# RoyAPTX4869/RaLD

Hardware: AMD Instinct MI355X
Metric: denoising steps/sec (whole node) (higher is better)
Workload: dtype bf16

## Files before the change

### include/rald_hip.h

```cpp
#ifndef RALD_HIP_H
#define RALD_HIP_H
#include <stdint.h>
#ifdef __cplusplus
extern "C" {
#endif

const char* rald_last_error(void);
int rald_version(void);
int rald_build_flags(void);
int64_t rald_debug_f16_saturation_count(int32_t reset);
int rald_debug_poison_lds(void* stream);

typedef struct rald_dit rald_dit;

typedef struct rald_dit_config {
    int32_t n_latents;
    int32_t channels;
    int32_t depth;
    int32_t n_heads;
    int32_t d_head;
    int32_t t_channels;
    int32_t context_dim;
    int32_t n_cond_tokens;
    int32_t with_radar_enc;
// ... 158 lines not shown
int64_t rald_radar_points_workspace_bytes(const rald_radar_points_config* cfg, int32_t batch);
int rald_radar_points_run(const rald_radar_points* h, const float* cubes, int32_t batch, float* points, int32_t* counts, int32_t* peaks,
                          float* intensities, void* workspace, int64_t workspace_bytes, void* stream);

typedef struct rald_lidar_config {
    double pc_range[6];
    double voxel_size[3];
    int32_t max_points_per_voxel, max_voxels, num_point_features;
    int32_t view_cone_mode, norm_anisotropy, norm_isotropy;
    double extrinsic[16];
    double fov[6];
} rald_lidar_config;
typedef struct rald_lidar rald_lidar;
int rald_lidar_create(const rald_lidar_config* cfg, rald_lidar** out);
void rald_lidar_destroy(rald_lidar* h);
int64_t rald_lidar_workspace_bytes(const rald_lidar_config* cfg, int32_t batch, int64_t total_points);
int rald_lidar_crop(const rald_lidar* h, const float* points, int32_t in_stride, const int64_t* offsets, int32_t batch, float* out,
                    int32_t* counts, void* workspace, int64_t workspace_bytes, void* stream);
int rald_lidar_voxelize(const rald_lidar* h, const float* points, const int64_t* offsets, const int32_t* counts, int32_t batch,
                        int32_t to_polar, float* polar_out, float* voxels, int32_t* coords, int32_t* num_points, int32_t* kept_keys,
                        int32_t* voxel_counts, void* workspace, int64_t workspace_bytes, void* stream);
int rald_lidar_queries(const rald_lidar* h, const float* points, const int64_t* offsets, int32_t batch, int32_t num_samples,
                       int32_t in_num, const int64_t* sample_idx, const double* u_in, const int64_t* voxel_idx, const double* u_out,
                       const int64_t* empty_rank, const int32_t* coords, const int32_t* kept_keys, const int32_t* voxel_counts,
                       float* lidar_points, float* query_points, float* query_labels, void* workspace, int64_t workspace_bytes,
                       void* stream);

int rald_op_gemm_nt(const void* A, int64_t lda, int64_t strideA, const void* B, int64_t ldb, int64_t strideB,
                    void* C, int64_t ldc, int64_t strideC, const float* bias, int32_t M, int32_t N, int32_t K,
                    int32_t batch, float alpha, int32_t epilogue, void* stream);
int rald_op_gemm_nt2(const void* A, int64_t lda, int64_t strideA, int64_t strideA2, const void* B, int64_t ldb, int64_t strideB, int64_t strideB2,
                     void* C, int64_t ldc, int64_t strideC, int64_t strideC2, const float* bias, int32_t M, int32_t N, int32_t K, int32_t batch,
                     int32_t batch2, float alpha, int32_t epilogue, void* stream);
int rald_op_gemm_tn(const void* A_bf16, int64_t lda, const void* B_bf16, int64_t ldb, float* C, int64_t ldc, float* colsum, int32_t M, int32_t N1,
                    int32_t N2, void* workspace, int64_t workspace_bytes, void* stream);
int rald_op_conv3d_wgrad(const void* dy_bf16, const void* x_bf16, float* dW, float* dbias, int32_t B, int32_t ID, int32_t IH, int32_t IW, int32_t Cin,
                         int32_t Cout, int32_t stride, int32_t pad, void* workspace, int64_t workspace_bytes, void* stream);
int64_t rald_op_gemm_tn_workspace_bytes(int32_t M, int32_t N1, int32_t N2);
int64_t rald_op_conv3d_wgrad_workspace_bytes(int32_t B, int32_t ID, int32_t IH, int32_t IW, int32_t Cin, int32_t Cout, int32_t stride, int32_t pad);
int rald_op_patches27(const float* cube, int32_t cube_ch, void* out_bf16, int32_t B, int32_t D, int32_t H, int32_t W, void* stream);
int rald_op_transpose(const void* in, int32_t in_is_bf16, int64_t ld_in, int64_t stride_in, int64_t stride_in2, void* out_bf16, int64_t ld_out,
                      int64_t stride_out, int64_t stride_out2, int32_t rows, int32_t cols, int32_t batch, int32_t batch2, void* stream);
int rald_op_ln_mod_bwd(const float* x, const float* dh, const float* scale, int64_t gstride, int32_t rows_per_group, float add_one, float eps,
                       int64_t rows, int32_t D, float* dx_accum, void* dx_bf16_out, float* dscale_accum, float* dshift_accum, void* stream);
int rald_op_geglu_fwd(const void* u_bf16, void* hid_bf16, int64_t M, int32_t inner, void* stream);
int rald_op_geglu_bwd(const void* u_bf16, const void* dhid_bf16, void* du_bf16, int64_t M, int32_t inner, void* stream);
int rald_op_colsum(const void* X, int32_t is_bf16, int64_t ld, int64_t M, int32_t N, float* out_accum, void* stream);
int rald_op_row_lse(const float* S, int64_t rows, int32_t cols, float scale, float* lse, void* stream);
int rald_op_rowdot_heads(const void* dO_bf16, const void* O_bf16, int64_t M, int32_t heads, int32_t nq, float* delta, void* stream);
int rald_op_attn_bwd_elem(const float* S, const float* dP, const float* lse, const float* delta, int64_t batch, int32_t R, int32_t Ccols,
                          int64_t vbatch_stride, int32_t vstride, float scale, int32_t by_col, void* P_bf16, void* dS_bf16, void* stream);
int rald_op_sgemm_acc(const float* A, int64_t lda, int32_t trans_a, const float* B, int64_t ldb, int32_t trans_b, float* C, int64_t ldc, int32_t M,
                      int32_t N, int32_t K, float alpha, void* stream);
int rald_op_silu_fwd(const float* x, float* y, int64_t n, void* stream);
int rald_op_silu_bwd(const float* x_pre, const float* dy, float* dx, int64_t n, void* stream);
int rald_op_posemb(const float* t, float* out, int32_t n, int32_t channels, void* stream);
int rald_op_edm_loss_grad(const float* F, const float* x_noised, const float* y, const float* coef3, int64_t per_sample, int64_t total, float* dF,
                          float* D_out, double* loss, void* stream);
int rald_op_conv3d(const void* in_bf16, const void* w_packed_bf16, const float* bias, const float* resid, float* out, void* out_bf16, int32_t B,
                   int32_t ID, int32_t IH, int32_t IW, int32_t Cin, int32_t Cout, int32_t stride, int32_t pad, void* stream);
int rald_op_conv3d_route(int32_t B, int32_t ID, int32_t IH, int32_t IW, int32_t Cin, int32_t Cout, int32_t stride, int32_t pad, int32_t allow_split,
                         int32_t* splits_out);
int rald_op_conv3d_full(const void* in_bf16, const void* w_packed_bf16, const float* bias, const float* resid, float* out, void* out_bf16,
                        double* gn_part, void* split_workspace, int64_t split_workspace_bytes, int32_t allow_split, int32_t B, int32_t ID,
                        int32_t IH, int32_t IW, int32_t Cin, int32_t Cout, int32_t stride, int32_t pad, void* stream);
int rald_op_gn_finish(const double* part, double* stats, int32_t B, int32_t nblk, void* stream);
// ... 117 lines not shown
```

### rald_amd/_handles.py

```python
from __future__ import annotations

import ctypes as C
import os
from typing import Dict, Iterable, Optional, Sequence, Tuple

import torch

from . import _lib
from ._lib import DitConfig, check, lib


def _stream() -> int:
    return torch.cuda.current_stream().cuda_stream


def _opt(t: Optional[torch.Tensor]) -> Optional[int]:
    return t.data_ptr() if t is not None else None


def _need_cuda(t: torch.Tensor, what: str) -> None:
    if not t.is_cuda:
        raise RuntimeError(f"rald_amd: {what} must live on the GPU (cuda tensor); this package has no CPU path")


# ... 296 lines not shown
def op_philox_normal(seeds: torch.Tensor, n_per_sample: int, tag: int = 0, step: int = 0, out: Optional[torch.Tensor] = None) -> torch.Tensor:
    _need_cuda(seeds, "seeds")
    if seeds.dtype != torch.int64 or seeds.dim() != 1:
        raise ValueError("seeds must be an int64 [B] tensor")
    seeds = seeds.contiguous()
    B = seeds.shape[0]
    if out is None:
        out = torch.empty(B, int(n_per_sample), device=seeds.device, dtype=torch.float32)
    assert out.dtype == torch.float32 and out.is_cuda and out.is_contiguous() and out.numel() == B * int(n_per_sample)
    check(lib().rald_op_philox_normal(seeds.data_ptr(), B, int(n_per_sample), int(tag), int(step), out.data_ptr(), _stream()))
    return out


def op_gemm_nt(A: torch.Tensor, B: torch.Tensor, bias: Optional[torch.Tensor] = None, epilogue: int = 0,
               C_inout: Optional[torch.Tensor] = None, alpha: float = 1.0) -> torch.Tensor:
    batched = A.dim() == 3 or B.dim() == 3
    batch = (A.shape[0] if A.dim() == 3 else B.shape[0]) if batched else 1
    M, K = A.shape[-2], A.shape[-1]
    N = B.shape[-2]
    sA = A.stride(0) if A.dim() == 3 else 0
    sB = B.stride(0) if B.dim() == 3 else 0
    nc = N // 2 if epilogue == 3 else N
    if epilogue == 2:
        out = C_inout
    else:
        shape = (batch, M, nc) if batched else (M, nc)
        out = torch.empty(shape, device=A.device, dtype=torch.float16 if epilogue == 5 else (torch.bfloat16 if epilogue in (0, 3, 4) else torch.float32))
    sC = out.stride(0) if out.dim() == 3 else 0
    check(lib().rald_op_gemm_nt(A.data_ptr(), A.stride(-2), sA, B.data_ptr(), B.stride(-2), sB, out.data_ptr(), out.stride(-2), sC, _opt(bias), M, N,
                                K, batch, alpha, epilogue, _stream()))
    return out


def op_gemm_tn(A: torch.Tensor, B: torch.Tensor, C_inout: torch.Tensor, colsum: Optional[torch.Tensor] = None, atomics: bool = True) -> torch.Tensor:
    M, N1 = A.shape
    N2 = B.shape[1]
    assert A.dtype == torch.bfloat16 and B.dtype == torch.bfloat16 and C_inout.dtype == torch.float32 and B.shape[0] == M
    assert A.stride(1) == 1 and B.stride(1) == 1 and C_inout.stride(1) == 1 and C_inout.shape == (N1, N2)
    ws, nbytes = None, 0
    if not atomics:
        nbytes = lib().rald_op_gemm_tn_workspace_bytes(M, N1, N2)
        ws = _scratch(nbytes, A.device)
    check(lib().rald_op_gemm_tn(A.data_ptr(), A.stride(0), B.data_ptr(), B.stride(0), C_inout.data_ptr(), C_inout.stride(0),
                                _opt(colsum), M, N1, N2, _opt(ws), nbytes, _stream()))
    return C_inout


def op_gemm_resid_ln(A: torch.Tensor, W: torch.Tensor, bias: torch.Tensor, x: torch.Tensor, g: torch.Tensor, b: torch.Tensor,
                     gstride: int = 0, rows_per_group: int = 1 << 30, add_one: float = 0.0, eps: float = 1e-5) -> torch.Tensor:
    M, K = A.shape
    h = torch.empty(M, 512, device=A.device, dtype=torch.bfloat16)
    check(lib().rald_op_gemm_resid_ln(A.data_ptr(), A.stride(0), W.data_ptr(), W.stride(0), bias.data_ptr(),
                                      x.data_ptr(), h.data_ptr(), g.data_ptr(), b.data_ptr(), gstride,
                                      rows_per_group, add_one, eps, M, K, _stream()))
    return h


def op_resid_gemm_ln(x: torch.Tensor, bias: torch.Tensor, M: int, K: int, A: Optional[torch.Tensor] = None, W: Optional[torch.Tensor] = None,
                     A8: Optional[torch.Tensor] = None, SA: Optional[torch.Tensor] = None, W8: Optional[torch.Tensor] = None,
                     SW: Optional[torch.Tensor] = None, h: Optional[torch.Tensor] = None, h8: Optional[torch.Tensor] = None,
                     hs: Optional[torch.Tensor] = None, g: Optional[torch.Tensor] = None, b: Optional[torch.Tensor] = None, gstride: int = 0,
                     rows_per_group: int = 1 << 30, add_one: float = 0.0, eps: float = 1e-5, strideW: int = 0, w_rows: int = 0, nt_io: int = 1,
                     route: int = 0, scratch: Optional[torch.Tensor] = None, lda: Optional[int] = None, ldw: Optional[int] = None) -> None:
    a, w = (A, W) if A is not None else (A8, W8)
    lda = a.stride(-2) if lda is None else lda
    ldw = w.stride(-2) if ldw is None else ldw
# ... 343 lines not shown
```

### rald_amd/csrc/api.hip

```cpp
#include <cstdlib>
#include <cstring>

#include "ae.h"
#include "dit.h"
#include "lidar.h"
#include "radar_dsp.h"
#include "radar_points.h"

using namespace rald;

struct rald_dit { Dit impl; };
struct rald_ae { Ae impl; };

extern "C" {

const char* rald_last_error(void) { return rald::last_error(); }
int rald_version(void) { return 3; }
int rald_build_flags(void) { return 0; }

int64_t rald_debug_f16_saturation_count(int32_t reset) {
    unsigned a = 0, b = 0;
    if (hipDeviceSynchronize() != hipSuccess) return -1;
    if (f16_saturation_gemm(&a, reset != 0) || f16_saturation_attn(&b, reset != 0)) return -1;
    return (int64_t)a + (int64_t)b;
// ... 465 lines not shown
int rald_optim_clip_coef(const double* sumsq, float pre_scale, float max_norm, float* out_norm_coef, void* stream) {
    RALD_CHECK(sumsq && out_norm_coef, "rald_optim_clip_coef: null argument");
    return optim_clip_coef(sumsq, pre_scale, max_norm, out_norm_coef, (hipStream_t)stream);
}
int rald_optim_adamw_ema(float* params, const float* grads, float* exp_avg, float* exp_avg_sq, float* ema_params, int64_t n,
                         const float* grad_scale, double lr, double beta1, double beta2, double eps, double weight_decay, int64_t step,
                         double ema_rate, int32_t write_back_grads, void* stream) {
    RALD_CHECK(n == 0 || (params && grads && exp_avg && exp_avg_sq), "rald_optim_adamw_ema: null argument");
    return optim_adamw_ema(params, grads, exp_avg, exp_avg_sq, ema_params, n, grad_scale, lr, beta1, beta2, eps, weight_decay, step, ema_rate,
                           write_back_grads, (hipStream_t)stream);
}
int rald_optim_ema(float* ema_params, const float* params, int64_t n, double rate, void* stream) {
    RALD_CHECK(n == 0 || (ema_params && params), "rald_optim_ema: null argument");
    return optim_ema(ema_params, params, n, rate, (hipStream_t)stream);
}

int rald_op_gemm_nt(const void* A, int64_t lda, int64_t strideA, const void* B, int64_t ldb, int64_t strideB,
                    void* C, int64_t ldc, int64_t strideC, const float* bias, int32_t M, int32_t N, int32_t K,
                    int32_t batch, float alpha, int32_t epilogue, void* stream) {
    RALD_CHECK(A && B && C, "rald_op_gemm_nt: null pointer");
    GemmArgs g;
    g.A = (const bf16*)A; g.lda = lda; g.strideA = strideA; g.B = (const bf16*)B; g.ldb = ldb; g.strideB = strideB;
    g.C = C; g.ldc = ldc; g.strideC = strideC; g.bias = bias; g.M = M; g.N = N; g.K = K; g.batch = batch; g.alpha = alpha; g.alpha_ncols = 1 << 30; g.flags = 0;
    return gemm_nt(g, epilogue, (hipStream_t)stream);
}
int rald_op_gemm_nt2(const void* A, int64_t lda, int64_t strideA, int64_t strideA2, const void* B, int64_t ldb, int64_t strideB, int64_t strideB2,
                     void* C, int64_t ldc, int64_t strideC, int64_t strideC2, const float* bias, int32_t M, int32_t N, int32_t K, int32_t batch,
                     int32_t batch2, float alpha, int32_t epilogue, void* stream) {
    RALD_CHECK(A && B && C, "rald_op_gemm_nt2: null pointer");
    GemmArgs g = gemm_args((const bf16*)A, lda, (const bf16*)B, ldb, C, ldc, bias, M, N, K);
    g.strideA = strideA; g.strideB = strideB; g.strideC = strideC; g.batch = batch; g.alpha = alpha;
    g.batch2 = batch2; g.strideA2 = strideA2; g.strideB2 = strideB2; g.strideC2 = strideC2;
    return gemm_nt(g, epilogue, (hipStream_t)stream);
}
int rald_op_gemm_tn(const void* A_bf16, int64_t lda, const void* B_bf16, int64_t ldb, float* C, int64_t ldc, float* colsum, int32_t M, int32_t N1,
                    int32_t N2, void* workspace, int64_t workspace_bytes, void* stream) {
    return gemm_tn((const bf16*)A_bf16, lda, (const bf16*)B_bf16, ldb, C, ldc, colsum, M, N1, N2, (hipStream_t)stream, (float*)workspace, workspace_bytes / 4);
}
int rald_op_conv3d_wgrad(const void* dy_bf16, const void* x_bf16, float* dW, float* dbias, int32_t B, int32_t ID, int32_t IH, int32_t IW, int32_t Cin,
                         int32_t Cout, int32_t stride, int32_t pad, void* workspace, int64_t workspace_bytes, void* stream) {
    return conv3d_wgrad_tn((const bf16*)dy_bf16, (const bf16*)x_bf16, dW, dbias, B, ID, IH, IW, Cin, Cout, stride, pad, (hipStream_t)stream, (float*)workspace,
                           workspace_bytes / 4);
}
int64_t rald_op_gemm_tn_workspace_bytes(int32_t M, int32_t N1, int32_t N2) { return 4 * gemm_tn_workspace_floats(M, N1, N2); }
int64_t rald_op_conv3d_wgrad_workspace_bytes(int32_t B, int32_t ID, int32_t IH, int32_t IW, int32_t Cin, int32_t Cout, int32_t stride, int32_t pad) {
    return 4 * conv3d_wgrad_workspace_floats(B, ID, IH, IW, Cin, Cout, stride, pad);
}
int rald_op_patches27(const float* cube, int32_t cube_ch, void* out_bf16, int32_t B, int32_t D, int32_t H, int32_t W, void* stream) {
    return patches27(cube, cube_ch, (bf16*)out_bf16, B, D, H, W, (hipStream_t)stream);
}
int rald_op_transpose(const void* in, int32_t in_is_bf16, int64_t ld_in, int64_t stride_in, int64_t stride_in2, void* out_bf16, int64_t ld_out,
                      int64_t stride_out, int64_t stride_out2, int32_t rows, int32_t cols, int32_t batch, int32_t batch2, void* stream) {
    TransposeArgs a;
    a.in = in; a.ld_in = ld_in; a.stride_in = stride_in; a.stride_in2 = stride_in2; a.out = (bf16*)out_bf16; a.ld_out = ld_out;
    a.stride_out = stride_out; a.stride_out2 = stride_out2; a.rows = rows; a.cols = cols; a.batch = batch; a.batch2 = batch2;
    return transpose_rows(a, in_is_bf16, (hipStream_t)stream);
}
int rald_op_ln_mod_bwd(const float* x, const float* dh, const float* scale, int64_t gstride, int32_t rows_per_group, float add_one, float eps,
                       int64_t rows, int32_t D, float* dx_accum, void* dx_bf16_out, float* dscale_accum, float* dshift_accum, void* stream) {
    RALD_CHECK(x && dh && scale && dx_accum && dscale_accum && dshift_accum, "rald_op_ln_mod_bwd: null pointer");
    return ln_mod_bwd(x, dh, scale, gstride, rows_per_group, add_one, eps, rows, D, dx_accum, dscale_accum, dshift_accum, (hipStream_t)stream, (bf16*)dx_bf16_out);
}
int rald_op_geglu_fwd(const void* u_bf16, void* hid_bf16, int64_t M, int32_t inner, void* stream) {
    RALD_CHECK(u_bf16 && hid_bf16, "rald_op_geglu_fwd: null pointer");
    return geglu_fwd((const bf16*)u_bf16, (bf16*)hid_bf16, M, inner, (hipStream_t)stream);
}
// ... 377 lines not shown
```

### rald_amd/csrc/gemm.hip

```cpp
#include <cstdlib>
#include <type_traits>

#include "common.h"
#include "kernels.h"
#include "gemm_epilogue.h"
#include "gemm_tile.h"

namespace rald {

template <int MT, int NT, int EPI>
__device__ __forceinline__ void gemm_epilogue(f32x4 (&acc)[MT][NT], const GemmArgs& a, int mb, int nb, int64_t coff, int fr, int fq) {
    if constexpr (EPI == EPI_GEGLU) {
        bf16* C = reinterpret_cast<bf16*>(a.C) + coff;
#pragma unroll
        for (int i = 0; i < MT; ++i) {
            const int m = mb + i * 16 + fr;
            if (m >= a.M) continue;
#pragma unroll
            for (int p = 0; p < NT / 2; ++p) {
                const int nx = nb + 32 * p + 4 * fq;
                const int ng = nx + 16;
                float4 bx = *reinterpret_cast<const float4*>(a.bias + nx);
                float4 bg = *reinterpret_cast<const float4*>(a.bias + ng);
                f32x4 x = acc[i][2 * p], g = acc[i][2 * p + 1];
                bf16x4 o = pack4((x[0] + bx.x) * gelu_erf(g[0] + bg.x), (x[1] + bx.y) * gelu_erf(g[1] + bg.y),
                                 (x[2] + bx.z) * gelu_erf(g[2] + bg.z), (x[3] + bx.w) * gelu_erf(g[3] + bg.w));
                const int c = nb / 2 + 16 * p + 4 * fq;
                *reinterpret_cast<bf16x4*>(C + (int64_t)m * a.ldc + c) = o;
            }
        }
    } else {
#pragma unroll
// ... 248 lines not shown
            __builtin_amdgcn_s_barrier();
        };
        for (int kt = 1; kt + 1 < nk; ++kt) body(kt, std::true_type{});
        if (nk > 1) body(nk - 1, std::false_type{});
        mfma_all(fa1, fb1);
    } else {
#pragma unroll
        for (int s = 0; s < NSTAGE - 1; ++s)
            if (s < nk) stage(s, s);
        for (int kt = 0; kt < nk; ++kt) {
            if (kt + NSTAGE - 2 < nk) asm volatile("s_waitcnt vmcnt(%0)" ::"n"((NSTAGE - 2) * (CA + CB)) : "memory");
            else asm volatile("s_waitcnt vmcnt(0)" ::: "memory");
            asm volatile("" ::: "memory");
            __builtin_amdgcn_s_barrier();
            asm volatile("" ::: "memory");
            if (kt + NSTAGE - 1 < nk) stage(kt + NSTAGE - 1, (kt + NSTAGE - 1) % NSTAGE);
#pragma unroll
            for (int kk = 0; kk < 2; ++kk) {
                bf16x8 fa[MT], fb[NT];
                read_frags(kt % NSTAGE, kk, fa, fb);
                mfma_all(fa, fb);
            }
        }
    }
    if constexpr (NSTAGE != 2) {
        asm volatile("" ::: "memory");
        __builtin_amdgcn_s_barrier();
        asm volatile("" ::: "memory");
    }
    gemm_epilogue_lds<MT, NT, EPI>(acc, a, m0 + wm * (BM / WM), n0 + wn * (BN / WN), coff, lane, smem + wave * EPI_PATCH_BYTES,
                                   reinterpret_cast<float*>(smem + WAVES * EPI_PATCH_BYTES) + wave * NT * 16);
}

template <int BM, int BN>
static int launch_tile(const GemmArgs& a, int epi, hipStream_t st) {
    dim3 grid(cdiv(a.N, BN), cdiv(a.M, BM), a.batch * a.batch2);
    switch (epi) {
        case EPI_BF16:  hipLaunchKernelGGL((gemm_nt_kernel<BM, BN, EPI_BF16>), grid, dim3(256), 0, st, a); break;
        case EPI_F32:   hipLaunchKernelGGL((gemm_nt_kernel<BM, BN, EPI_F32>), grid, dim3(256), 0, st, a); break;
        case EPI_RESID: hipLaunchKernelGGL((gemm_nt_kernel<BM, BN, EPI_RESID>), grid, dim3(256), 0, st, a); break;
        case EPI_GEGLU: hipLaunchKernelGGL((gemm_nt_kernel<BM, BN, EPI_GEGLU>), grid, dim3(256), 0, st, a); break;
        default: set_error("gemm: bad epilogue"); return 1;
    }
    RALD_HIP(hipGetLastError());
    return 0;
}

template <int BM, int BN, int WM, int WN, int NSTAGE, int EPI>
static int launch_glds_epi(const GemmArgs& a, hipStream_t st) {
    constexpr int WAVES = WM * WN;
    constexpr int smem = NSTAGE * (BM + BN) * 64 * 2;
    static_assert(smem >= epi_lds_bytes<BN / (16 * WN)>(WAVES), "epilogue patches and bias slots must fit in the staging buffers");
    static bool raised = false;
    return launch_dyn_lds(gemm_nt_glds_kernel<BM, BN, WM, WN, NSTAGE, EPI>, raised, dim3(cdiv(a.N, BN), cdiv(a.M, BM), a.batch * a.batch2), WAVES * 64, smem, st, a);
}
template <int BM, int BN, int WM, int WN, int NSTAGE>
static int launch_glds(const GemmArgs& a, int epi, hipStream_t st) {
    switch (epi) {
        case EPI_BF16:  return launch_glds_epi<BM, BN, WM, WN, NSTAGE, EPI_BF16>(a, st);
        case EPI_F32:   return launch_glds_epi<BM, BN, WM, WN, NSTAGE, EPI_F32>(a, st);
        case EPI_RESID: return launch_glds_epi<BM, BN, WM, WN, NSTAGE, EPI_RESID>(a, st);
        case EPI_GEGLU: return launch_glds_epi<BM, BN, WM, WN, NSTAGE, EPI_GEGLU>(a, st);
        case EPI_F16S:
            if constexpr ((BM == 64 && BN == 64) || (BM == 128 && BN == 128 && NSTAGE == 2)) return launch_glds_epi<BM, BN, WM, WN, NSTAGE, EPI_F16S>(a, st);
            else { set_error("gemm: the fp16-slab epilogue is built for the 64x64 ring and the 128x128 LDS-DMA engines"); return 1; }
        case EPI_SOFTMAX64:
            if constexpr ((BN / WN) % 64 == 0 && BM >= 128) return launch_glds_epi<BM, BN, WM, WN, NSTAGE, EPI_SOFTMAX64>(a, st);
            else { set_error("gemm: the softmax epilogue needs waves of 64-column groups"); return 1; }
        default: set_error("gemm: bad epilogue"); return 1;
    }
}

int f16_saturation_gemm(unsigned* count, bool reset) {
    RALD_HIP(hipMemcpyFromSymbol(count, HIP_SYMBOL(g_f16_sat_gemm), sizeof(unsigned)));
    if (reset) { const unsigned z = 0; RALD_HIP(hipMemcpyToSymbol(HIP_SYMBOL(g_f16_sat_gemm), &z, sizeof(unsigned))); }
    return 0;
}

int gemm_nt(const GemmArgs& a0, int epi, hipStream_t st) {
    GemmArgs a = a0;
    a.flags |= GEMM_NT_STORE;
    RALD_CHECK(a.M > 0 && a.N > 0 && a.K > 0 && a.batch > 0 && a.batch2 > 0, "gemm: empty problem");
    const int64_t nbatch = (int64_t)a.batch * a.batch2;
    RALD_CHECK(nbatch <= 65535, "gemm: batch * batch2 exceeds the grid z limit");
    RALD_CHECK(a.K % 64 == 0, "gemm: K must be a multiple of 64 (pad with zeros)");
    RALD_CHECK(a.N % 4 == 0, "gemm: N must be a multiple of 4");
    RALD_CHECK(a.lda % 8 == 0 && a.ldb % 8 == 0, "gemm: lda/ldb must be multiples of 8 elements (16-byte rows)");
    RALD_CHECK(a.lda >= a.K && a.ldb >= a.K, "gemm: leading dimension smaller than K");
    RALD_CHECK(((uintptr_t)a.A % 16 == 0) && ((uintptr_t)a.B % 16 == 0) && ((uintptr_t)a.C % 16 == 0), "gemm: pointers must be 16-byte aligned");
    RALD_CHECK(a.ldc % 4 == 0, "gemm: ldc must be a multiple of 4");
    if (epi == EPI_GEGLU) {
        RALD_CHECK(a.N % 128 == 0 && a.bias != nullptr, "gemm: GEGLU needs N % 128 == 0 and a packed bias");
        RALD_CHECK(a.ldc >= a.N / 2, "gemm: GEGLU ldc < N/2");
    } else {
        RALD_CHECK(a.ldc >= a.N, "gemm: ldc < N");
    }
    if (epi == EPI_F16S) {
        RALD_CHECK(!a.out8 && a.N % 8 == 0, "gemm: the fp16-slab epilogue needs N % 8 == 0");
        const int64_t w128 = (int64_t)cdiv(a.M, 128) * cdiv(a.N, 128) * nbatch, w64 = (int64_t)cdiv(a.M, 64) * cdiv(a.N, 64) * nbatch;
        RALD_CHECK(w128 >= 192 || w64 <= 256, "gemm: fp16 slabs are not built for the register-staged engine (ask gemm_f16s_ok first)");
        if (w128 >= 192) return launch_glds<128, 128, 2, 2, 2>(a, epi, st);
        return launch_glds<64, 64, 2, 2, 8>(a, epi, st);
    }
    if (epi == EPI_SOFTMAX64) {
        RALD_CHECK(a.M % 128 == 0 && a.N % 128 == 0 && !a.bias && !a.out8 && a.alpha_ncols >= a.N, "gemm: the softmax epilogue needs M, N % 128 == 0 and no bias");
        if (a.M % 256 == 0 && a.N % 256 == 0 && (int64_t)(a.M / 256) * (a.N / 256) * nbatch >= 256) return launch_glds<256, 256, 4, 2, 2>(a, epi, st);
        return launch_glds<128, 128, 2, 2, 2>(a, epi, st);
    }
    if (a.out8) {
        RALD_CHECK(epi == EPI_GEGLU && a.outs && a.batch * a.batch2 == 1 && a.M % 256 == 0 && a.N % 256 == 0 && (a.N / 2) % 32 == 0 &&
                   (int64_t)(a.M / 256) * (a.N / 256) >= 256, "gemm: the MXFP8 output form needs the GEGLU epilogue on full 256x256 tiles");
        return launch_glds<256, 256, 4, 2, 2>(a, epi, st);
    }
    const int64_t wg128 = (int64_t)cdiv(a.M, 128) * cdiv(a.N, 128) * nbatch;
    if (wg128 < 192) {
        const int64_t wg64 = (int64_t)cdiv(a.M, 64) * cdiv(a.N, 64) * nbatch;
        if (wg64 > 256) return launch_tile<64, 64>(a, epi, st);
        return launch_glds<64, 64, 2, 2, 8>(a, epi, st);
    }
    const int64_t wg256 = (int64_t)(a.M / 256) * (a.N / 256) * nbatch;
    if (a.M % 256 == 0 && a.N % 256 == 0 && wg256 >= 256) return launch_glds<256, 256, 4, 2, 2>(a, epi, st);
    if (epi != EPI_GEGLU && wg128 <= 320 && a.M % 64 == 0) return launch_glds<64, 128, 2, 2, 3>(a, epi, st);
    return launch_glds<128, 128, 2, 2, 2>(a, epi, st);
}

}
```

### rald_amd/csrc/gemm_tile.h

```cpp
#pragma once
#include "common.h"

namespace rald {

typedef int i32x8 __attribute__((ext_vector_type(8)));
typedef int i32x4 __attribute__((ext_vector_type(4)));

#define RALD_SWZ(row, chunk) ((chunk) ^ ((row) & 7))

__device__ __forceinline__ void xcd_strip_tile(int& tm, int& tn) {
    const int ntn = gridDim.x, ntm = gridDim.y, nt = ntn * ntm;
    const int lin = blockIdx.y * gridDim.x + blockIdx.x;
    const int xcd = lin & 7, q = nt >> 3, rr = nt & 7;
    const int tile = (xcd < rr ? xcd * (q + 1) : rr * (q + 1) + (xcd - rr) * q) + (lin >> 3);
    constexpr int GN = 8;
    if (ntn % GN == 0) {
        const int strip = tile / (ntm * GN), within = tile % (ntm * GN);
        tm = within / GN;
        tn = strip * GN + within % GN;
    } else {
        tm = tile / ntn;
        tn = tile % ntn;
    }
}

template <int WAVES, typename T, int C>
__device__ __forceinline__ void dma_sources(const T* (&g)[C], const T* base, int64_t ld, int row0, int rows, int wave, int lane) {
    const int lr = lane >> 3;
    const int lc = RALD_SWZ(lr, lane & 7);
#pragma unroll
    for (int p = 0; p < C; ++p) {
        int r = row0 + 8 * (wave + WAVES * p) + lr;
        r = r < rows ? r : rows - 1;
        g[p] = base + (int64_t)r * ld + lc * (16 / (int)sizeof(T));
    }
}
template <int BM, int WAVES, typename T, int CA, int CB>
__device__ __forceinline__ void dma_stage(const T* const (&gA)[CA], const T* const (&gB)[CB], int kt, int nk, unsigned char* stage, int wave) {
    constexpr int BK = 128 / (int)sizeof(T);
    const int koff = 0;
    int ks = kt + koff;
    ks = ks >= nk ? ks - nk : ks;
#pragma unroll
    for (int p = 0; p < CA; ++p)
        __builtin_amdgcn_global_load_lds((glb_void*)(gA[p] + ks * BK), (lds_void*)(stage + (wave + WAVES * p) * 1024), 16, 0, 0);
#pragma unroll
    for (int p = 0; p < CB; ++p)
        __builtin_amdgcn_global_load_lds((glb_void*)(gB[p] + ks * BK), (lds_void*)(stage + BM * 128 + (wave + WAVES * p) * 1024), 16, 0, 0);
}

__device__ __forceinline__ i32x8 frag_mx8(const unsigned char* tile, int row, int fq) {
    const i32x4* s = reinterpret_cast<const i32x4*>(tile) + row * 8;
    const i32x4 lo = s[RALD_SWZ(row, fq)], hi = s[RALD_SWZ(row, fq + 4)];
    return i32x8{lo[0], lo[1], lo[2], lo[3], hi[0], hi[1], hi[2], hi[3]};
}

// ... 84 lines not shown
```

### rald_amd/csrc/kernels.h

```cpp
#pragma once
#include <cstdlib>
#include <vector>

#include "common.h"

namespace rald {

enum { GEMM_NT_STORE = 64 };
enum { EPI_BF16 = 0, EPI_F32 = 1, EPI_RESID = 2, EPI_GEGLU = 3,
       EPI_SOFTMAX64 = 4,
       EPI_F16S = 5 };
struct GemmArgs {
    const bf16* A; int64_t lda; int64_t strideA;
    const bf16* B; int64_t ldb; int64_t strideB;
    void* C;       int64_t ldc; int64_t strideC;
    const float* bias;
    int M, N, K, batch;
    float alpha;
    int alpha_ncols;
    int flags;
    int batch2 = 1;
    int64_t strideA2 = 0, strideB2 = 0, strideC2 = 0;
    unsigned char *out8 = nullptr, *outs = nullptr;
};
#ifdef __HIPCC__
__device__ __forceinline__ void gemm_batch_offsets(const GemmArgs& a, int bz, int64_t& oa, int64_t& ob, int64_t& oc) {
    const int b1 = bz / a.batch2, b2 = bz - b1 * a.batch2;
    oa = (int64_t)b1 * a.strideA + (int64_t)b2 * a.strideA2;
    ob = (int64_t)b1 * a.strideB + (int64_t)b2 * a.strideB2;
    oc = (int64_t)b1 * a.strideC + (int64_t)b2 * a.strideC2;
}
#endif
int gemm_nt(const GemmArgs& a, int epi, hipStream_t st);
int f16_saturation_gemm(unsigned* count, bool reset);
int f16_saturation_attn(unsigned* count, bool reset);
inline bool gemm_f16s_ok(int M, int N, int batch) {
    const int64_t w128 = (int64_t)((M + 127) / 128) * ((N + 127) / 128) * batch, w64 = (int64_t)((M + 63) / 64) * ((N + 63) / 64) * batch;
    return w128 >= 192 || w64 <= 256;
}
inline GemmArgs gemm_args(const bf16* A, int64_t lda, const bf16* B, int64_t ldb, void* C, int64_t ldc,
                          const float* bias, int M, int N, int K) {
    GemmArgs g;
    g.A = A; g.lda = lda; g.strideA = 0; g.B = B; g.ldb = ldb; g.strideB = 0;
    g.C = C; g.ldc = ldc; g.strideC = 0; g.bias = bias; g.M = M; g.N = N; g.K = K; g.batch = 1; g.alpha = 1.f; g.alpha_ncols = 1 << 30; g.flags = 0;
    return g;
}

struct GemmLnArgs {
    const bf16* A; int64_t lda;
    const bf16* W; int64_t ldw;
    const float* bias;
    float* x;
    bf16* h;
    unsigned char* h8 = nullptr;
    unsigned char* hs = nullptr;
    int nt_io = 1;
    const unsigned char *A8 = nullptr, *SA = nullptr, *W8 = nullptr, *SW = nullptr;
    const float* g; const float* b; int64_t gstride; int rows_per_group; float add_one, eps;
    int M, K;
    int64_t strideW = 0; int w_rows = 1 << 30;
};
int gemm_resid_ln(const GemmLnArgs& a, hipStream_t st);
inline bool gemm_resid_ln_pays(int M, int K = 512) { (void)K; return M >= 16384; }
inline GemmLnArgs gemm_ln_args(const bf16* A, int64_t lda, const bf16* W, int64_t ldw, const float* bias, float* x, bf16* h,
                               const float* g, const float* b, int64_t gstride, int rows_per_group, float add_one, int M, int K) {
    GemmLnArgs a;
// ... 270 lines not shown
```

Baseline: 5659.

## Add persistent 256x256 GEMM kernel that prefetches the next tile during the epilogue

Adds a persistent bf16 GEMM kernel (256x256 tiles, 8 waves, half of them issuing direct-to-LDS loads) that loops over output tiles. It starts loading the next tile's first K stages before running the current tile's epilogue, which stages output through LDS. gemm_nt routes single-batch BF16/GEGLU problems with at least two tiles per CU to this kernel instead of the non-persistent 256x256 path. This aims to remove per-tile launch and prologue cost and to hide epilogue stores behind the next tile's loads. In exchange it adds hand-scheduled code that needs a large LDS allocation, plus a test entry point.

```diff
diff --git a/include/rald_hip.h b/include/rald_hip.h
--- a/include/rald_hip.h
+++ b/include/rald_hip.h
@@ -214,6 +214,8 @@
 int rald_op_gemm_nt2(const void* A, int64_t lda, int64_t strideA, int64_t strideA2, const void* B, int64_t ldb, int64_t strideB, int64_t strideB2,
                      void* C, int64_t ldc, int64_t strideC, int64_t strideC2, const float* bias, int32_t M, int32_t N, int32_t K, int32_t batch,
                      int32_t batch2, float alpha, int32_t epilogue, void* stream);
+int rald_op_gemm_nt_256(const void* A, int64_t lda, const void* B, int64_t ldb, void* C, int64_t ldc, const float* bias, int32_t M, int32_t N,
+                        int32_t K, float alpha, int32_t alpha_ncols, int32_t epilogue, int32_t persistent, int32_t max_workgroups, void* stream);
 int rald_op_gemm_tn(const void* A_bf16, int64_t lda, const void* B_bf16, int64_t ldb, float* C, int64_t ldc, float* colsum, int32_t M, int32_t N1,
                     int32_t N2, void* workspace, int64_t workspace_bytes, void* stream);
 int rald_op_conv3d_wgrad(const void* dy_bf16, const void* x_bf16, float* dW, float* dbias, int32_t B, int32_t ID, int32_t IH, int32_t IW, int32_t Cin,
diff --git a/rald_amd/_handles.py b/rald_amd/_handles.py
--- a/rald_amd/_handles.py
+++ b/rald_amd/_handles.py
@@ -352,6 +352,16 @@
     return out
 
 
+def op_gemm_nt_256(A: torch.Tensor, B: torch.Tensor, out: torch.Tensor, bias: Optional[torch.Tensor] = None, epilogue: int = 0, alpha: float = 1.0,
+                   alpha_ncols: int = 1 << 30, persistent: int = 1, max_workgroups: int = 1 << 30) -> torch.Tensor:
+    (M, K), N = A.shape, B.shape[0]
+    assert A.dtype == B.dtype == out.dtype == torch.bfloat16 and A.stride(1) == B.stride(1) == out.stride(1) == 1
+    assert out.shape == (M, N // 2 if epilogue == 3 else N) and B.shape[1] == K
+    check(lib().rald_op_gemm_nt_256(A.data_ptr(), A.stride(0), B.data_ptr(), B.stride(0), out.data_ptr(), out.stride(0), _opt(bias), M, N, K,
+                                    alpha, int(alpha_ncols), int(epilogue), int(persistent), int(max_workgroups), _stream()))
+    return out
+
+
 def op_gemm_tn(A: torch.Tensor, B: torch.Tensor, C_inout: torch.Tensor, colsum: Optional[torch.Tensor] = None, atomics: bool = True) -> torch.Tensor:
     M, N1 = A.shape
     N2 = B.shape[1]
diff --git a/rald_amd/csrc/api.hip b/rald_amd/csrc/api.hip
--- a/rald_amd/csrc/api.hip
+++ b/rald_amd/csrc/api.hip
@@ -521,6 +521,13 @@
     g.strideA = strideA; g.strideB = strideB; g.strideC = strideC; g.batch = batch; g.alpha = alpha;
     g.batch2 = batch2; g.strideA2 = strideA2; g.strideB2 = strideB2; g.strideC2 = strideC2;
     return gemm_nt(g, epilogue, (hipStream_t)stream);
+}
+int rald_op_gemm_nt_256(const void* A, int64_t lda, const void* B, int64_t ldb, void* C, int64_t ldc, const float* bias, int32_t M, int32_t N,
+                        int32_t K, float alpha, int32_t alpha_ncols, int32_t epilogue, int32_t persistent, int32_t max_workgroups, void* stream) {
+    RALD_CHECK(A && B && C, "rald_op_gemm_nt_256: null pointer");
+    GemmArgs g = gemm_args((const bf16*)A, lda, (const bf16*)B, ldb, C, ldc, bias, M, N, K);
+    g.alpha = alpha; g.alpha_ncols = alpha_ncols;
+    return gemm_nt_256_test(g, epilogue, persistent, max_workgroups, (hipStream_t)stream);
 }
 int rald_op_gemm_tn(const void* A_bf16, int64_t lda, const void* B_bf16, int64_t ldb, float* C, int64_t ldc, float* colsum, int32_t M, int32_t N1,
                     int32_t N2, void* workspace, int64_t workspace_bytes, void* stream) {
diff --git a/rald_amd/csrc/gemm.hip b/rald_amd/csrc/gemm.hip
--- a/rald_amd/csrc/gemm.hip
+++ b/rald_amd/csrc/gemm.hip
@@ -1,3 +1,4 @@
+#include <algorithm>
 #include <cstdlib>
 #include <type_traits>
 
@@ -312,6 +313,221 @@
                                    reinterpret_cast<float*>(smem + WAVES * EPI_PATCH_BYTES) + wave * NT * 16);
 }
 
+constexpr int PERSIST_LDS_BYTES = 160 * 1024;
+template <int EPI>
+__global__ __launch_bounds__(512) void gemm_nt_persist_kernel(GemmArgs a) {
+    static_assert(EPI == EPI_BF16 || EPI == EPI_GEGLU, "the persistent engine is built for the two bf16-output epilogues");
+    constexpr int BM = 256, BN = 256, BK = 64, WN = 2, MT = 4, NT = 8;
+    constexpr int DW = 4;
+    constexpr int CP = BM / 8 / DW;
+    constexpr int STAGE_BYTES = (BM + BN) * BK * 2;
+    constexpr int OC = (EPI == EPI_GEGLU) ? NT * 8 : NT * 16;
+    constexpr int ROWB = OC * 2, STRIDE = ROWB + 16, LPR = ROWB / 16;
+    constexpr int PR = (EPI == EPI_GEGLU) ? 16 : 8;
+    constexpr int PATCH = PR * STRIDE;
+    constexpr int RPI = 64 / LPR;
+    constexpr int BIAS_OFF = 2 * STAGE_BYTES + 31 * 1024;
+    static_assert(2 * STAGE_BYTES + 8 * PATCH <= BIAS_OFF && BIAS_OFF + BN * 4 <= PERSIST_LDS_BYTES && PR % RPI == 0, "LDS plan");
+    extern __shared__ __attribute__((aligned(16))) unsigned char smem[];
+    float* tbias = reinterpret_cast<float*>(smem + BIAS_OFF);
+
+    const int tid = threadIdx.x;
+    const int lane = tid & 63;
+    const int wave = __builtin_amdgcn_readfirstlane(tid >> 6);
+    const int wm = wave / WN, wn = wave % WN;
+    const bool dma = wave < DW;
+    const int ntm = a.M / BM, ntn = a.N / BN, nt = ntm * ntn;
+    const int nk = a.K / BK;
+    const int fr = lane & 15, fq = lane >> 4;
+
+    const unsigned voA = (unsigned)((lane >> 3) * (int)a.lda + RALD_SWZ(lane >> 3, lane & 7) * 8) * 2u;
+    const unsigned voB = (unsigned)((lane >> 3) * (int)a.ldb + RALD_SWZ(lane >> 3, lane & 7) * 8) * 2u;
+    const unsigned lds0 = (unsigned)(uintptr_t)(lds_void*)smem;
+    auto dma_piece = [&](const char* base, unsigned voff, unsigned lds) {
+        asm volatile("s_nop 0\n\tglobal_load_lds_dwordx4 %0, %1" ::"v"(voff), "s"(base), "{m0}"(lds) : "memory");
+    };
+    auto stage = [&](int m0, int n0, int kt, int buf) {
+        const char* pa = reinterpret_cast<const char*>(a.A) + ((int64_t)(m0 + 8 * wave) * a.lda + kt * BK) * 2;
+        const char* pb = reinterpret_cast<const char*>(a.B) + ((int64_t)(n0 + 8 * wave) * a.ldb + kt * BK) * 2;
+        const unsigned s = lds0 + buf * STAGE_BYTES + wave * 1024;
+#pragma unroll
+        for (int p = 0; p < CP; ++p) dma_piece(pa + (int64_t)p * (8 * DW * 2) * a.lda, voA, s + p * DW * 1024);
+#pragma unroll
+        for (int p = 0; p < CP; ++p) dma_piece(pb + (int64_t)p * (8 * DW * 2) * a.ldb, voB, s + BM * 128 + p * DW * 1024);
+    };
+    auto read_frags = [&](int buf, int kk, bf16x8 (&fa)[MT], bf16x8 (&fb)[NT]) {
+        const bf16x8* sA = reinterpret_cast<const bf16x8*>(smem + buf * STAGE_BYTES);
+        const bf16x8* sB = sA + BM * 8;
+        const int chunk = kk * 4 + fq;
+#pragma unroll
+        for (int i = 0; i < MT; ++i) {
+            const int r = wm * (MT * 16) + i * 16 + fr;
+            fa[i] = sA[r * 8 + RALD_SWZ(r, chunk)];
+        }
+#pragma unroll
+        for (int j = 0; j < NT; ++j) {
+            const int r = wn * (NT * 16) + j * 16 + fr;
+            fb[j] = sB[r * 8 + RALD_SWZ(r, chunk)];
+        }
+    };
+    f32x4 acc[MT][NT];
+    auto mfma_all = [&](const bf16x8 (&fa)[MT], const bf16x8 (&fb)[NT]) {
+#pragma unroll
+        for (int i = 0; i < MT; ++i)
+#pragma unroll
+            for (int j = 0; j < NT; ++j)
+                acc[i][j] = __builtin_amdgcn_mfma_f32_16x16x32_bf16(fb[j], fa[i], acc[i][j], 0, 0, 0);
+    };
+    constexpr int W_ALL = 0x0070;
+    constexpr int W_LGKM = 0xc07f;
+    constexpr int W_ST1 = ((2 * CP) & 15) | (((2 * CP) >> 4) << 14) | 0x0070;
+    auto hand_over = [&]() {
+        if (dma) __builtin_amdgcn_s_waitcnt(W_ALL);
+        else __builtin_amdgcn_s_waitcnt(W_LGKM);
+        __builtin_amdgcn_s_barrier();
+    };
+    bf16x8 fa0[MT], fb0[NT], fa1[MT], fb1[NT];
+    auto body = [&](int m0, int n0, int kt, bool with_dma) {
+        const int cur = kt & 1;
+        if (with_dma && dma) stage(m0, n0, kt + 1, cur ^ 1);
+        __builtin_amdgcn_sched_barrier(0);
+        read_frags(cur, 0, fa0, fb0);
+        mfma_all(fa1, fb1);
+#pragma unroll
+        for (int g = 0; g < 12; ++g) {
+            __builtin_amdgcn_sched_group_barrier(0x008, 2, 0);
+            __builtin_amdgcn_sched_group_barrier(0x100, 1, 0);
+        }
+        __builtin_amdgcn_sched_group_barrier(0x008, 8, 0);
+        __builtin_amdgcn_sched_barrier(0);
+        read_frags(cur, 1, fa1, fb1);
+        mfma_all(fa0, fb0);
+#pragma unroll
+        for (int g = 0; g < 12; ++g) {
+            __builtin_amdgcn_sched_group_barrier(0x008, 2, 0);
+            __builtin_amdgcn_sched_group_barrier(0x100, 1, 0);
+        }
+        __builtin_amdgcn_sched_group_barrier(0x008, 8, 0);
+        __builtin_amdgcn_sched_barrier(0);
+        hand_over();
+    };
+
+    if (!a.bias && tid < BN / 4) *reinterpret_cast<float4*>(tbias + 4 * tid) = make_float4(0.f, 0.f, 0.f, 0.f);
+    int t = blockIdx.x;
+    int tm, tn;
+    xcd_strip_tile_at(t, ntn, ntm, tm, tn);
+    int m0 = tm * BM, n0 = tn * BN;
+    if (dma) {
+        stage(m0, n0, 0, 0);
+        if (nk > 1) stage(m0, n0, 1, 1);
+    }
+    for (;;) {
+#pragma unroll
+        for (int i = 0; i < MT; ++i)
+#pragma unroll
+            for (int j = 0; j < NT; ++j) acc[i][j] = f32x4{0.f, 0.f, 0.f, 0.f};
+        if (dma) {
+            if (nk > 1) __builtin_amdgcn_s_waitcnt(W_ST1);
+            else __builtin_amdgcn_s_waitcnt(W_ALL);
+        } else __builtin_amdgcn_s_waitcnt(W_LGKM);
+        __builtin_amdgcn_s_barrier();
+        if (wave == 0 && a.bias) dma_piece(reinterpret_cast<const char*>(a.bias + n0), 16u * lane, lds0 + BIAS_OFF);
+        read_frags(0, 0, fa0, fb0);
+        read_frags(0, 1, fa1, fb1);
+        mfma_all(fa0, fb0);
+        hand_over();
+        for (int kt = 1; kt + 1 < nk; ++kt) body(m0, n0, kt, true);
+        if (nk > 1) body(m0, n0, nk - 1, false);
+        const int tnext = t + gridDim.x;
+        int m0n = 0, n0n = 0;
+        if (tnext < nt) {
+            xcd_strip_tile_at(tnext, ntn, ntm, tm, tn);
+            m0n = tm * BM;
+            n0n = tn * BN;
+            if (dma) {
+                stage(m0n, n0n, 0, 0);
+                if (nk > 1) stage(m0n, n0n, 1, 1);
+            }
+        }
+        mfma_all(fa1, fb1);
+
+        {
+            int lane_e = lane;
+            asm volatile("" : "+v"(lane_e));
+            const int fr = lane_e & 15, fq = lane_e >> 4;
+            unsigned char* patch = smem + 2 * STAGE_BYTES + wave * PATCH;
+            const int mb = m0 + wm * (MT * 16), nb = n0 + wn * (NT * 16);
+            const int oc0 = (EPI == EPI_GEGLU) ? nb / 2 : nb;
+            const float* wbias = tbias + wn * (NT * 16);
+            bf16* C = reinterpret_cast<bf16*>(a.C);
+#pragma unroll
+            for (int i = 0; i < MT; ++i) {
+#pragma unroll
+                for (int h = 0; h < 16 / PR; ++h) {
+                    asm volatile("" ::: "memory");
+                    if (PR == 16 || (fr >> 3) == h) {
+                        const int pr = fr & (PR - 1);
+                        if constexpr (EPI == EPI_GEGLU) {
+#pragma unroll
+                            for (int p = 0; p < NT / 2; ++p) {
+                                const float4 bx = *reinterpret_cast<const float4*>(wbias + 32 * p + 4 * fq);
+                                const float4 bg = *reinterpret_cast<const float4*>(wbias + 32 * p + 4 * fq + 16);
+                                const f32x4 x = acc[i][2 * p], g = acc[i][2 * p + 1];
+                                const f32x2 g01 = gelu_poly2(f32x2{g[0] + bg.x, g[1] + bg.y});
+                                const f32x2 g23 = gelu_poly2(f32x2{g[2] + bg.z, g[3] + bg.w});
+                                const f32x2 o01 = f32x2{x[0] + bx.x, x[1] + bx.y} * g01;
+                                const f32x2 o23 = f32x2{x[2] + bx.z, x[3] + bx.w} * g23;
+                                *reinterpret_cast<bf16x4*>(patch + pr * STRIDE + (16 * p + 4 * fq) * 2) = pack4(o01[0], o01[1], o23[0], o23[1]);
+                            }
+                        } else {
+#pragma unroll
+                            for (int j = 0; j < NT; ++j) {
+                                const int n = nb + j * 16 + 4 * fq;
+                                const float4 b = *reinterpret_cast<const float4*>(wbias + 16 * j + 4 * fq);
+                                const f32x4 v = acc[i][j];
+                                const float al = n < a.alpha_ncols ? a.alpha : 1.0f;
+                                const float o0 = al * v[0] + b.x, o1 = al * v[1] + b.y, o2 = al * v[2] + b.z, o3 = al * v[3] + b.w;
+                                *reinterpret_cast<bf16x4*>(patch + pr * STRIDE + (16 * j + 4 * fq) * 2) = pack4(o0, o1, o2, o3);
+                            }
+                        }
+                    }
+                    asm volatile("" ::: "memory");
+                    __builtin_amdgcn_s_waitcnt(W_LGKM);
+                    __builtin_amdgcn_s_barrier();
+                    asm volatile("" ::: "memory");
+                    if (!dma) {
+                        const int r = lane_e / LPR, pc = lane_e % LPR;
+                        uint4 v[2][PR / RPI];
+#pragma unroll
+                        for (int w2 = 0; w2 < 2; ++w2)
+#pragma unroll
+                            for (int q = 0; q < PR / RPI; ++q)
+                                v[w2][q] = *reinterpret_cast<const uint4*>(patch - w2 * DW * PATCH + (q * RPI + r) * STRIDE + pc * 16);
+#pragma unroll
+                        for (int w2 = 0; w2 < 2; ++w2)
+#pragma unroll
+                            for (int q = 0; q < PR / RPI; ++q) {
+                                const int m = mb - w2 * (BM / 2) + i * 16 + h * PR + q * RPI + r;
+                                bf16* Cp = C + (int64_t)m * a.ldc + oc0 + pc * 8;
+                                typedef unsigned int u32x4 __attribute__((ext_vector_type(4)));
+                                const u32x4 vv = u32x4{v[w2][q].x, v[w2][q].y, v[w2][q].z, v[w2][q].w};
+                                asm volatile("global_store_dwordx4 %0, %1, off sc0 sc1 nt\n\ts_nop 1" ::"v"(Cp), "v"(vv) : "memory");
+                            }
+                    }
+                    asm volatile("" ::: "memory");
+                    __builtin_amdgcn_s_waitcnt(W_LGKM);
+                    __builtin_amdgcn_s_barrier();
+                    asm volatile("" ::: "memory");
+                }
+            }
+        }
+        if (tnext >= nt) break;
+        t = tnext;
+        m0 = m0n;
+        n0 = n0n;
+    }
+}
+
 template <int BM, int BN>
 static int launch_tile(const GemmArgs& a, int epi, hipStream_t st) {
     dim3 grid(cdiv(a.N, BN), cdiv(a.M, BM), a.batch * a.batch2);
@@ -348,6 +564,29 @@
             if constexpr ((BN / WN) % 64 == 0 && BM >= 128) return launch_glds_epi<BM, BN, WM, WN, NSTAGE, EPI_SOFTMAX64>(a, st);
             else { set_error("gemm: the softmax epilogue needs waves of 64-column groups"); return 1; }
         default: set_error("gemm: bad epilogue"); return 1;
+    }
+}
+
+static int cu_count(int& cus) {
+    static int cached[64] = {};
+    int dev = 0;
+    RALD_HIP(hipGetDevice(&dev));
+    RALD_CHECK(dev >= 0 && dev < 64, "gemm: device index out of range");
+    if (cached[dev] == 0) RALD_HIP(hipDeviceGetAttribute(&cached[dev], hipDeviceAttributeMultiprocessorCount, dev));
+    cus = cached[dev];
+    return 0;
+}
+static int launch_persist(const GemmArgs& a, int epi, int max_workgroups, hipStream_t st) {
+    int cus = 0;
+    if (int rc = cu_count(cus)) return rc;
+    const int64_t tiles = (int64_t)(a.M / 256) * (a.N / 256);
+    const int grid = (int)std::min<int64_t>(tiles, std::min(cus, max_workgroups));
+    RALD_CHECK(grid >= 1, "gemm: the persistent engine needs at least one workgroup");
+    static bool raised_bf16 = false, raised_geglu = false;
+    switch (epi) {
+        case EPI_BF16:  return launch_dyn_lds(gemm_nt_persist_kernel<EPI_BF16>, raised_bf16, dim3(grid), 512, PERSIST_LDS_BYTES, st, a);
+        case EPI_GEGLU: return launch_dyn_lds(gemm_nt_persist_kernel<EPI_GEGLU>, raised_geglu, dim3(grid), 512, PERSIST_LDS_BYTES, st, a);
+        default: set_error("gemm: the persistent engine has the bf16 and GEGLU epilogues"); return 1;
     }
 }
 
@@ -399,9 +638,32 @@
         return launch_glds<64, 64, 2, 2, 8>(a, epi, st);
     }
     const int64_t wg256 = (int64_t)(a.M / 256) * (a.N / 256) * nbatch;
-    if (a.M % 256 == 0 && a.N % 256 == 0 && wg256 >= 256) return launch_glds<256, 256, 4, 2, 2>(a, epi, st);
+    if (a.M % 256 == 0 && a.N % 256 == 0 && wg256 >= 256) {
+        if (nbatch == 1 && (epi == EPI_BF16 || epi == EPI_GEGLU)) {
+            int cus = 0;
+            if (int rc = cu_count(cus)) return rc;
+            if (wg256 >= 2 * (int64_t)cus) return launch_persist(a, epi, 1 << 30, st);
+        }
+        return launch_glds<256, 256, 4, 2, 2>(a, epi, st);
+    }
     if (epi != EPI_GEGLU && wg128 <= 320 && a.M % 64 == 0) return launch_glds<64, 128, 2, 2, 3>(a, epi, st);
     return launch_glds<128, 128, 2, 2, 2>(a, epi, st);
 }
 
-}
+int gemm_nt_256_test(const GemmArgs& a0, int epi, int persistent, int max_workgroups, hipStream_t st) {
+    GemmArgs a = a0;
+    a.flags |= GEMM_NT_STORE;
+    RALD_CHECK(epi == EPI_BF16 || epi == EPI_GEGLU, "gemm_nt_256_test: EPI_BF16 or EPI_GEGLU");
+    RALD_CHECK(a.M > 0 && a.N > 0 && a.K > 0 && a.M % 256 == 0 && a.N % 256 == 0 && a.K % 64 == 0, "gemm_nt_256_test: M, N % 256 == 0 and K % 64 == 0");
+    RALD_CHECK(a.batch == 1 && a.batch2 == 1 && !a.out8, "gemm_nt_256_test: one problem, bf16 output");
+    RALD_CHECK(a.lda % 8 == 0 && a.ldb % 8 == 0 && a.lda >= a.K && a.ldb >= a.K, "gemm_nt_256_test: lda/ldb must be multiples of 8 and at least K");
+    RALD_CHECK(((uintptr_t)a.A % 16 == 0) && ((uintptr_t)a.B % 16 == 0) && ((uintptr_t)a.C % 16 == 0) && ((uintptr_t)a.bias % 16 == 0),
+               "gemm_nt_256_test: pointers must be 16-byte aligned");
+    RALD_CHECK(a.ldc % 8 == 0 && a.ldc >= (epi == EPI_GEGLU ? a.N / 2 : a.N), "gemm_nt_256_test: ldc");
+    RALD_CHECK(epi != EPI_GEGLU || a.bias, "gemm_nt_256_test: GEGLU needs a packed bias");
+    RALD_CHECK(max_workgroups >= 1, "gemm_nt_256_test: max_workgroups must be at least 1");
+    if (persistent) return launch_persist(a, epi, max_workgroups, st);
+    return launch_glds<256, 256, 4, 2, 2>(a, epi, st);
+}
+
+}
diff --git a/rald_amd/csrc/gemm_tile.h b/rald_amd/csrc/gemm_tile.h
--- a/rald_amd/csrc/gemm_tile.h
+++ b/rald_amd/csrc/gemm_tile.h
@@ -8,9 +8,8 @@
 
 #define RALD_SWZ(row, chunk) ((chunk) ^ ((row) & 7))
 
-__device__ __forceinline__ void xcd_strip_tile(int& tm, int& tn) {
-    const int ntn = gridDim.x, ntm = gridDim.y, nt = ntn * ntm;
-    const int lin = blockIdx.y * gridDim.x + blockIdx.x;
+__device__ __forceinline__ void xcd_strip_tile_at(int lin, int ntn, int ntm, int& tm, int& tn) {
+    const int nt = ntn * ntm;
     const int xcd = lin & 7, q = nt >> 3, rr = nt & 7;
     const int tile = (xcd < rr ? xcd * (q + 1) : rr * (q + 1) + (xcd - rr) * q) + (lin >> 3);
     constexpr int GN = 8;
@@ -22,6 +21,9 @@
         tm = tile / ntn;
         tn = tile % ntn;
     }
+}
+__device__ __forceinline__ void xcd_strip_tile(int& tm, int& tn) {
+    xcd_strip_tile_at(blockIdx.y * gridDim.x + blockIdx.x, gridDim.x, gridDim.y, tm, tn);
 }
 
 template <int WAVES, typename T, int C>
diff --git a/rald_amd/csrc/kernels.h b/rald_amd/csrc/kernels.h
--- a/rald_amd/csrc/kernels.h
+++ b/rald_amd/csrc/kernels.h
@@ -32,6 +32,7 @@
 }
 #endif
 int gemm_nt(const GemmArgs& a, int epi, hipStream_t st);
+int gemm_nt_256_test(const GemmArgs& a, int epi, int persistent, int max_workgroups, hipStream_t st);
 int f16_saturation_gemm(unsigned* count, bool reset);
 int f16_saturation_attn(unsigned* count, bool reset);
 inline bool gemm_f16s_ok(int M, int N, int batch) {
```

Result: faster. 5820 (median of 6 runs) (+2.8%).
